# monatis/clip.cpp

Measured on AMD Instinct MI355X. Metric: image+text embeddings/sec, higher is better.
Workload: dtype f16

## Files before the change

### clip_cpp_amd/csrc/forward.cpp

```cpp
#include <cmath>
#include <cstdio>
#include <cstdlib>
#include <cstring>
#include <thread>
#include <utility>

#include "model.h"

namespace clipamd {

namespace {

constexpr size_t kGuardBytes = 4096;
constexpr int kGuardByte = 0xA5;
bool guard_mode() {
    static const bool on = [] { const char * e = getenv("CLIP_AMD_GUARD"); return e && e[0] == '1'; }();
    return on;
}

struct Carver {
    uint8_t * base;
    size_t off = 0;
    std::vector<size_t> * gaps = nullptr;
    explicit Carver(void * b, std::vector<size_t> * g = nullptr) : base((uint8_t *)b), gaps(g) { if (gaps) gaps->clear(); }
// ... 28 lines not shown
    std::vector<uint8_t> h(kGuardBytes);
    bool ok = true;
    for (size_t i = 0; i < ctx->guard_gaps.size(); i++) {
        if (hipMemcpy(h.data(), (uint8_t *)ctx->ws.base + ctx->guard_gaps[i], kGuardBytes, hipMemcpyDeviceToHost) != hipSuccess) return false;
        for (size_t k = 0; k < kGuardBytes; k++)
            if (h[k] != (uint8_t)kGuardByte) {
                fprintf(stderr, "%s: CLIP_AMD_GUARD: workspace buffer %zu was written %zu bytes past its end\n", who, i, k);
                ok = false;
                break;
            }
    }
    return ok;
}

struct ProfScope {
    clip_ctx * ctx;
    hipEvent_t a = nullptr, b = nullptr;
    bool on;
    std::string tag;
    double flops, bytes;
    ProfScope(clip_ctx * c, const char * family, long m, long n, long k, double fl, double by) : ctx(c), on(c->profiling), flops(fl), bytes(by) {
        if (!on) return;
        char buf[96];
        snprintf(buf, sizeof buf, "%s:%ldx%ldx%ld", family, m, n, k);
        tag = buf;
        (void)hipEventCreate(&a);
        (void)hipEventCreate(&b);
        (void)hipEventRecord(a, ctx->stream);
    }
    ~ProfScope() {
        if (!on) return;
        (void)hipEventRecord(b, ctx->stream);
        ctx->pending.push_back({a, b, tag, flops, bytes});
    }
};

double weight_bytes(const DevWeight & W) {
    const double nblk = (double)(W.K / 32) * W.N;
    switch (W.wtype) {
    case W_F16: return (double)W.N * W.K * 2;
    case W_Q4_0: return nblk * 18;
    case W_Q4_1: return nblk * 20;
    case W_Q5_0: return nblk * 22;
    case W_Q5_1: return nblk * 24;
    case W_Q8_0: return nblk * 34;
    case W_F32: return (double)W.N * W.K * 4;
    }
    return 0;
}

bool acts_f32(const clip_ctx * ctx, const DevTower & tw) {
    return ctx->f32_acts && !tw.layers.empty() && tw.layers[0].qkv.wtype == W_F32 && tw.layers[0].o.wtype == W_F32 && tw.layers[0].ff1.wtype == W_F32 && tw.layers[0].ff2.wtype == W_F32 &&
           tw.proj.wtype == W_F32;
}
void layernorm_act(bool f32, const float * x, int ldx, const int * in_rows, int in_row_mul, const float * w, const float * b, float eps, int rows, int h, half_t * dst,
                   hipStream_t s) {
    if (f32) launch_layernorm(x, ldx, in_rows, in_row_mul, w, b, eps, rows, h, nullptr, 0, (float *)dst, h, s);
    else launch_layernorm(x, ldx, in_rows, in_row_mul, w, b, eps, rows, h, dst, h, nullptr, 0, s);
}

bool device_shared(const clip_ctx * ctx) { return ctx->device_shared || ctx->sibling_busy || ctx->owner != nullptr; }

void gemm(clip_ctx * ctx, const char * what, const GemmParams & p0, int epi) {
    GemmParams p = p0;
    p.shared_device = device_shared(ctx);
    p.sk_ws = ctx->sk_ws; p.sk_ws_floats = ctx->sk_ws_floats; p.sk_cnt = ctx->sk_cnt; p.sk_cnt_n = ctx->sk_cnt_n;
    if (!ctx->profiling) {
        launch_gemm(p, epi, 0, ctx->stream);
        return;
    }
    const int wt = p.w16_pre ? (int)W_F16 : p.W.wtype;
    const int tile = gemm_tile_for(p.M, p.W.N, p.W.Kpad, wt != W_F16, p.shared_device);
    const bool panel = gemm_tile_uses_panel(tile) && wt == W_F16;
    const double fl = 2.0 * p.M * (double)p.W.N * p.W.K;
    const double wb = wt == W_F16 ? (double)p.W.N * p.W.K * 2 : weight_bytes(p.W);
    const double by = wb + (double)p.M * p.W.K * 2 + (double)p.M * p.W.N * (epi == EPI_F16 || epi == EPI_GELU_F16 || epi == EPI_QGELU_F16 ? 2 : epi == EPI_RESID_F32 ? 8 : 4)
                      + (p.xg_out ? (double)p.M * p.W.N * 2 : 0.0);
    char fam[96];
    if (wt == W_F32) snprintf(fam, sizeof fam, "gemm_f32_kernel<%d>/%s", epi, what);
    else if (panel && tile % 1000 == 261 && (epi == EPI_F16 || epi == EPI_GELU_F16 || epi == EPI_QGELU_F16)) snprintf(fam, sizeof fam, "gemm32_kernel<%d,4,%d>/%s", tile / 1000 == 320 ? 5 : 4, epi, what);
    else if (panel && tile % 1000 >= 259) snprintf(fam, sizeof fam, "gemm4_kernel<%d>/%s", epi, what);
    else if (panel) snprintf(fam, sizeof fam, "gemm8_kernel<%d,%d>/%s", tile / 32000, epi, what);
    else if (gemm_tile_is_ring(tile)) snprintf(fam, sizeof fam, "gemm_ring_kernel<%d,%d,4,%d,%d>/%s", wt, tile % 1000, tile % 1000 >= 128 ? 4 : 2, epi, what);
    else snprintf(fam, sizeof fam, "gemm_dma_kernel<%d,%d,%d,%d>/%s", wt, gemm_tile_uses_panel(tile) ? 160 : tile / 1000, gemm_tile_uses_panel(tile) ? 128 : tile % 1000, epi, what);
    ProfScope ps(ctx, fam, p.M, p.W.N, p.W.K, fl, by);
    launch_gemm(p, epi, 0, ctx->stream);
}

struct LayerPanels { const half_t * qkv = nullptr, * o = nullptr, * ff1 = nullptr, * ff2 = nullptr; };

bool ensure_panel(clip_ctx * ctx, size_t halfs) {
    if (ctx->w16_panel_halfs >= halfs) return true;
    (void)hipStreamSynchronize(ctx->stream);
    if (ctx->w16_panel) (void)hipFree(ctx->w16_panel);
    ctx->w16_panel = nullptr;
    ctx->w16_panel_halfs = 0;
    if (hipMalloc((void **)&ctx->w16_panel, halfs * sizeof(half_t)) != hipSuccess) { (void)hipGetLastError(); return false; }
    ctx->w16_panel_halfs = halfs;
    return true;
}

bool wants_resident_panel(const clip_ctx * ctx, const DevWeight & w, int i, int rows) {
    if (w.wtype == W_F16 || w.wtype == W_F32) return false;
    if (i == 3) return rows >= 4096 && gemm_tile_uses_panel(gemm_tile_for(rows, w.N, w.Kpad, false));
    if (i == 1) return rows >= 4096 && rows < 32768 && gemm_tile_uses_panel(gemm_tile_for(rows, w.N, w.Kpad, false));
    return rows >= 32768 && gemm_tile_for(rows, w.N, w.Kpad, false, device_shared(ctx)) % 1000 == 261;
}

LayerPanels dequant_layer(clip_ctx * ctx, const DevLayer & l, int rows, const half_t * const * res = nullptr) {
    LayerPanels lp;
    const DevWeight * ws[4] = {&l.qkv, &l.o, &l.ff1, &l.ff2};
    const half_t ** slot[4] = {&lp.qkv, &lp.o, &lp.ff1, &lp.ff2};
    const DevWeight * jw[4];
    half_t * jo[4];
    int nj = 0;
    size_t need = 0;
    bool todo[4];
    for (int i = 0; i < 4; i++) {
        if (res && res[i] && wants_resident_panel(ctx, *ws[i], i, rows)) { *slot[i] = res[i]; todo[i] = false; continue; }
        todo[i] = ws[i]->wtype != W_F16 && ws[i]->wtype != W_F32 && gemm_tile_uses_panel(gemm_tile_for(rows, ws[i]->N, ws[i]->Kpad, true));
        if (todo[i]) need += (size_t)ws[i]->Npad * ws[i]->Kpad;
    }
    if (!need || !ensure_panel(ctx, need)) return lp;
    size_t off = 0;
    for (int i = 0; i < 4; i++)
        if (todo[i]) {
            jw[nj] = ws[i];
            jo[nj] = ctx->w16_panel + off;
            *slot[i] = jo[nj];
            off += (size_t)ws[i]->Npad * ws[i]->Kpad;
            nj++;
        }
    ProfScope ps(ctx, "dequant_layer", rows, nj, 0, 0, (double)need * 2.5625);
    launch_dequant(jw, jo, nj, ctx->stream);
    return lp;
}

bool skinny_enabled() {
    static int on = -1;
    if (on < 0) { const char * e = getenv("CLIP_AMD_SKINNY"); on = !(e && e[0] == '0'); }
    return on != 0;
}

#ifdef CLIPAMD_SK_TIMING
unsigned long long * g_sk_stamps = nullptr;
int g_sk_stamp_launch = 0;
constexpr int SK_STAMP_LAUNCHES = 512;
#endif

void skinny(clip_ctx * ctx, const char * what, const SkinnyParams & p0, int epi) {
#ifdef CLIPAMD_SK_TIMING
    SkinnyParams p = p0;
    if (!g_sk_stamps && hipMalloc((void **)&g_sk_stamps, SK_STAMP_LAUNCHES * 16 * 8) == hipSuccess) (void)hipMemset(g_sk_stamps, 0, SK_STAMP_LAUNCHES * 16 * 8);
    if (g_sk_stamps) p.stamps = g_sk_stamps + (size_t)(g_sk_stamp_launch++ % SK_STAMP_LAUNCHES) * 16;
#else
    const SkinnyParams & p = p0;
#endif
    if (!ctx->profiling) { launch_skinny(p, epi, ctx->stream); return; }
    char fam[96];
    const int nw = (!p.x32 && p.W.Kpad >= 2048 && (epi == EPI_RESID_F32 || epi == EPI_PATCH_F32)) ? 8 : 4;
    snprintf(fam, sizeof fam, "skinny_kernel<%d,1,%d,%d,%s>/%s", p.W.wtype, nw, epi, p.x32 ? "true" : "false", what);
    const double fl = 2.0 * p.M * (double)p.W.N * p.W.K;
    const double by = weight_bytes(p.W) + (double)p.M * p.W.K * (p.x32 ? 4 : 2) + (double)p.M * p.W.N * (epi == EPI_RESID_F32 ? 8 : epi == EPI_F32 || epi == EPI_PATCH_F32 ? 4 : 2);
    ProfScope ps(ctx, fam, p.M, p.W.N, p.W.K, fl, by);
    launch_skinny(p, epi, ctx->stream);
}
// ... 767 lines not shown
```

### clip_cpp_amd/csrc/k_gemm.hip

```cpp

#include <vector>

#include "gemm_common.h"

namespace clipamd {

namespace {

constexpr int NTHREADS = 256;

constexpr bool gemm_tile_splits_k(int bm, int bn) { return bm == 64 && bn > 0; }

template <int WT, int BM, int BN, int EPI>
__global__ void __launch_bounds__(NTHREADS, ((BM + BN) * BK * 4 <= 80 * 1024 ? 2 : 1)) gemm_dma_kernel(const GemmParams p) {
    extern __shared__ __attribute__((aligned(16))) unsigned char smem_raw[];
    half_t * Xs = (half_t *)smem_raw;
    half_t * Ws = Xs + 2 * BM * BK;
    constexpr int TN = BN / 32, TM = BM / 32;
    constexpr int XPW = BM / 32;
    constexpr int WPW = BN / 32;

    const int tid = threadIdx.x;
    const int lane = tid & 63;
    const int wave = __builtin_amdgcn_readfirstlane(tid >> 6);
    const int wn = wave >> 1, wm = wave & 1;
    const int frow = lane & 15, fgrp = lane >> 4;

    const int tiles_m = (p.M + BM - 1) / BM;
    const int tiles_n = (p.W.N + BN - 1) / BN;
    constexpr bool SK = gemm_tile_splits_k(BM, BN);
    const int nwg = tiles_m * tiles_n * (SK ? p.ksplit : 1);
    int bid = blockIdx.x;
    {
        const int q = nwg >> 3, r = nwg & 7;
        const int xcd = bid & 7, idx = bid >> 3;
        bid = (xcd < r ? xcd * (q + 1) : r * (q + 1) + (xcd - r) * q) + idx;
    }
    const int ksplit = SK ? p.ksplit : 1;
    const int tile_id = SK ? bid / ksplit : bid;
    const int split = SK ? bid - tile_id * ksplit : 0;
    const int tile_n = tile_id % tiles_n, tile_m = tile_id / tiles_n;
    const int m0 = tile_m * BM, n0 = tile_n * BN;
    const int nk_all = p.W.Kpad / BK;
    const int kbeg = SK ? (split * nk_all) / ksplit : 0;
    const int nk = SK ? ((split + 1) * nk_all) / ksplit - kbeg : nk_all;
    const int last = nk - 1;

    const int prow = lane >> 3;
    const int pchunk = (lane & 7) ^ prow;
    const half_t * xsrc[XPW];
#pragma unroll
    for (int i = 0; i < XPW; i++) {
        int gm = m0 + (wave * XPW + i) * 8 + prow;
        gm = gm < p.M ? gm : p.M - 1;
        xsrc[i] = p.A + (size_t)gm * p.lda + pchunk * 8 + kbeg * BK;
    }
    const half_t * wsrc[WT == W_F16 ? WPW : 1];
    if constexpr (WT == W_F16) {
#pragma unroll
        for (int i = 0; i < WPW; i++)
            wsrc[i] = (const half_t *)p.W.w16 + (size_t)(n0 + (wave * WPW + i) * 8 + prow) * p.W.Kpad + pchunk * 8 + kbeg * BK;
    }
    constexpr int NB = (BN * 2 + NTHREADS - 1) / NTHREADS;
    RawBlock<WT> B0[NB], B1[NB];
    const int bnl = tid % BN, bkb = tid / BN;
    const bool bact = (BN * 2 >= NTHREADS) || tid < BN * 2;

#define DMA_TILE(buf_, kt_)                                                                    \
    {                                                                                          \
        _Pragma("unroll") for (int i = 0; i < XPW; i++)                                        \
            __builtin_amdgcn_global_load_lds((const __attribute__((address_space(1))) void *)(xsrc[i] + (kt_) * BK), \
                (__attribute__((address_space(3))) void *)(Xs + (buf_) * BM * BK + (wave * XPW + i) * 512), 16, 0, 0); \
        if constexpr (WT == W_F16) {                                                           \
            _Pragma("unroll") for (int i = 0; i < WPW; i++)                                    \
                __builtin_amdgcn_global_load_lds((const __attribute__((address_space(1))) void *)(wsrc[i] + (kt_) * BK), \
                    (__attribute__((address_space(3))) void *)(Ws + (buf_) * BN * BK + (wave * WPW + i) * 512), 16, 0, 0); \
        }                                                                                      \
    }
#define LOAD_B(B, kt_)                                                                         \
    if constexpr (WT != W_F16) {                                                               \
        if (bact) {                                                                            \
            _Pragma("unroll") for (int i_ = 0; i_ < NB; i_++)                                  \
                load_block<WT>(B[i_], p.W, (size_t)(((kt_) + kbeg) * 2 + bkb + i_ * (NTHREADS / BN)) * p.W.Npad + n0 + bnl); \
        }                                                                                      \
    }
#define STORE_B(B, buf_)                                                                       \
    if constexpr (WT != W_F16) {                                                               \
        if (bact) {                                                                            \
            half_t * wrow_ = Ws + (buf_) * BN * BK + bnl * BK;                                 \
            _Pragma("unroll") for (int i_ = 0; i_ < NB; i_++)                                  \
                _Pragma("unroll") for (int j = 0; j < 4; j++)                                  \
                    *(h8 *)(wrow_ + ((((bkb + i_ * (NTHREADS / BN)) * 4 + j) ^ (bnl & 7)) << 3)) = dequant_wfrag<WT>(block_word<WT>(B[i_], j), j); \
        }                                                                                      \
    }
    f4 acc[TN][TM];
#pragma unroll
    for (int a = 0; a < TN; a++)
#pragma unroll
// ... 127 lines not shown
    if (kt < nk) COMPUTE(0);
    }
#undef STEP_ILV
#undef FRAG
#undef DMA_TILE
#undef LOAD_B
#undef STORE_B
#undef COMPUTE
#undef COMPUTE_SCHED
    asm volatile("" ::: "memory");
#ifdef CLIPAMD_ABLATION
    if (p.debug & 8) {
        float keep = 0.f;
#pragma unroll
        for (int a = 0; a < TN; a++)
#pragma unroll
            for (int b = 0; b < TM; b++) keep += (acc[a][b][0] + acc[a][b][1]) + (acc[a][b][2] + acc[a][b][3]);
        if (keep == 1.2345e33f) ((float *)p.out)[tid] = keep;
        return;
    }
#endif
    if constexpr (SK) {
        if (ksplit > 1) {
            __shared__ int is_last;
            typedef unsigned long long u64;
            u64 * part = (u64 *)(p.sk_ws + ((size_t)tile_id * ksplit) * (BM * BN));
            constexpr int PER_SPLIT = BM * BN / 2;
#pragma unroll
            for (int a = 0; a < TN; a++)
#pragma unroll
                for (int b = 0; b < TM; b++) {
                    const float2 lo = make_float2(acc[a][b][0], acc[a][b][1]), hi = make_float2(acc[a][b][2], acc[a][b][3]);
                    u64 * dst = part + (size_t)split * PER_SPLIT + ((a * TM + b) * 2) * NTHREADS + tid;
                    __hip_atomic_store(dst, __builtin_bit_cast(u64, lo), __ATOMIC_RELAXED, __HIP_MEMORY_SCOPE_AGENT);
                    __hip_atomic_store(dst + NTHREADS, __builtin_bit_cast(u64, hi), __ATOMIC_RELAXED, __HIP_MEMORY_SCOPE_AGENT);
                }
            asm volatile("s_waitcnt vmcnt(0)" ::: "memory");
            __syncthreads();
            if (tid == 0) {
                const unsigned ticket = __hip_atomic_fetch_add(p.sk_cnt + tile_id, 1u, __ATOMIC_RELAXED, __HIP_MEMORY_SCOPE_AGENT);
                is_last = (ticket == (unsigned)ksplit - 1u);
                if (is_last) __hip_atomic_store(p.sk_cnt + tile_id, 0u, __ATOMIC_RELAXED, __HIP_MEMORY_SCOPE_AGENT);
            }
            __syncthreads();
            if (!is_last) return;
#pragma unroll
            for (int a = 0; a < TN; a++)
#pragma unroll
                for (int b = 0; b < TM; b++) acc[a][b] = (f4){0.f, 0.f, 0.f, 0.f};
            for (int sp = 0; sp < ksplit; sp++) {
#pragma unroll
                for (int a = 0; a < TN; a++)
#pragma unroll
                    for (int b = 0; b < TM; b++) {
                        const u64 * src = part + (size_t)sp * PER_SPLIT + ((a * TM + b) * 2) * NTHREADS + tid;
                        const float2 lo = __builtin_bit_cast(float2, __hip_atomic_load(src, __ATOMIC_RELAXED, __HIP_MEMORY_SCOPE_AGENT));
                        const float2 hi = __builtin_bit_cast(float2, __hip_atomic_load(src + NTHREADS, __ATOMIC_RELAXED, __HIP_MEMORY_SCOPE_AGENT));
                        acc[a][b] += (f4){lo.x, lo.y, hi.x, hi.y};
                    }
            }
        }
    }
    float2 * ln_rs = (float2 *)(smem_raw + ((BM * 272 + 15) & ~15));
    if constexpr (LNE) {
        if (ln) ln_rows_publish(ln_rs, ln_mine, tid, BM, [] { __syncthreads(); });
    }
    const float2 * rs_lane = ln_rs + wm * (BM / 2) + frow;
    if constexpr ((EPI == EPI_F16 || EPI == EPI_GELU_F16 || EPI == EPI_QGELU_F16) && BN == 128 && BM >= 128) {
        const int nb = n0 + wn * (BN / 2);
        if (nb + BN / 2 <= p.W.N && (p.ldc & 7) == 0) {
            if ((nk & 1) && !ln) __syncthreads();
            gemm_epilogue_f16_staged<EPI, TN, TM>(p, acc, nb, m0 + wm * (BM / 2), frow, fgrp, (half_t *)smem_raw + wave * (BM / 2) * 68, lane, ln, rs_lane);
            return;
        }
    }
    if constexpr (EPI == EPI_RESID_F32 && BN == 128 && BM >= 128) {
        if (p.xg_out) {
            if (nk & 1) __syncthreads();
            gemm_epilogue<EPI, TN, TM>(p, acc, n0 + wn * (BN / 2), m0 + wm * (BM / 2), frow, fgrp, false, rs_lane, (half_t *)smem_raw + wave * (BM / 2) * 68, lane);
            return;
        }
    }
    gemm_epilogue<EPI, TN, TM>(p, acc, n0 + wn * (BN / 2), m0 + wm * (BM / 2), frow, fgrp, ln, rs_lane);
}

template <int WT, int BM, int BN, int EPI>
void launch_dma(const GemmParams & p, hipStream_t stream) {
    const int tiles_m = (p.M + BM - 1) / BM, tiles_n = (p.W.N + BN - 1) / BN;
    constexpr size_t smem = (size_t)2 * (BM + BN) * BK * sizeof(half_t);
    static unsigned long long lds_ok = 0;
    if (smem > 64 * 1024) opt_in_dynamic_lds(gemm_dma_kernel<WT, BM, BN, EPI>, smem, lds_ok);
    int grid = tiles_m * tiles_n;
    if (gemm_tile_splits_k(BM, BN)) grid *= p.ksplit;
    hipLaunchKernelGGL((gemm_dma_kernel<WT, BM, BN, EPI>), dim3(grid), dim3(NTHREADS), smem, stream, p);
}

template <int WT, int EPI>
void launch_tile(const GemmParams & p, int tile, hipStream_t stream) {
    switch (tile % 1000000) {
    case 128128: launch_dma<WT, 128, 128, EPI>(p, stream); break;
    case 160128: launch_dma<WT, 160, 128, EPI>(p, stream); break;
    case 192128: launch_dma<WT, 192, 128, EPI>(p, stream); break;
#ifdef CLIPAMD_BIGTILES
    case 128256: launch_dma<WT, 128, 256, EPI>(p, stream); break;
    case 160256: launch_dma<WT, 160, 256, EPI>(p, stream); break;
    case 192256: launch_dma<WT, 192, 256, EPI>(p, stream); break;
    case 256256: launch_dma<WT, 256, 256, EPI>(p, stream); break;
#endif
    case 64128: launch_dma<WT, 64, 128, EPI>(p, stream); break;
    case 128064: launch_dma<WT, 128, 64, EPI>(p, stream); break;
    default: launch_dma<WT, 64, 64, EPI>(p, stream); break;
    }
}

template <int WT>
void launch_epi(const GemmParams & p, int epi, int tile, hipStream_t stream) {
    switch (epi) {
    case EPI_F32: launch_tile<WT, EPI_F32>(p, tile, stream); break;
    case EPI_F16: launch_tile<WT, EPI_F16>(p, tile, stream); break;
    case EPI_GELU_F16: launch_tile<WT, EPI_GELU_F16>(p, tile, stream); break;
    case EPI_QGELU_F16: launch_tile<WT, EPI_QGELU_F16>(p, tile, stream); break;
    case EPI_RESID_F32: launch_tile<WT, EPI_RESID_F32>(p, tile, stream); break;
    case EPI_PATCH_F32: launch_tile<WT, EPI_PATCH_F32>(p, tile, stream); break;
    }
}

int tile_override(int M, int N, int Kpad) {
#if !CLIPAMD_TEST_HOOKS
    (void)M; (void)N; (void)Kpad;
    return 0;
#else
    struct Ov { int M, N, K, tile; };
    static const std::vector<Ov> ovs = [] {
        std::vector<Ov> v;
        const char * e = getenv("CLIP_AMD_TILE_OVERRIDE");
        while (e && *e) {
            Ov o;
            int used = 0;
            if (sscanf(e, "%d,%d,%d,%d%n", &o.M, &o.N, &o.K, &o.tile, &used) == 4) v.push_back(o); else break;
            e += used;
            if (*e == ';') e++;
        }
        return v;
    }();
    for (const Ov & o : ovs) if (o.M == M && o.N == N && (o.K == 0 || o.K == Kpad)) return o.tile;
    return 0;
#endif
}

int pick_tile(int M, int N, int Kpad, bool quantised, bool shared = false) {
    auto wgs = [&](int bm, int bn) { return ((M + bm - 1) / bm) * ((N + bn - 1) / bn); };
    if (const int ov = tile_override(M, N, Kpad)) return ov;
    if (M <= 64) return 64064;
    if (M <= 4096) {
        const int tm = (M + 63) / 64, t64 = tm * ((N + 63) / 64), t128 = tm * ((N + 127) / 128), nk = Kpad / BK;
        if (nk < 32) {
            if (t64 <= 260) return 65064;
            if (t128 <= 500) return 65128;
        } else if (!quantised) {
            if (t64 <= 340) return 65064;
        } else if (M >= 1024 && t128 <= 340) {
            return 65128;
        }
    }
    if (wgs(128, 128) < 100) return wgs(64, 128) >= 256 ? 64128 : 64064;
    if (!shared && !quantised && M >= 32768 && N >= 3 * Kpad && (N & 63) == 0 && Kpad >= 128 && wgs(320, 256) >= 3 * 256) return 320261;
    if (M >= 32768 && wgs(256, 256) >= 2 * 256) return 256260;
    if (!shared && !quantised && M >= 8192 && N >= 2 * Kpad && (N & 63) == 0 && Kpad >= 128) {
        const int t4 = wgs(256, 256), t5 = wgs(320, 256);
        const int c4 = ((t4 + 255) / 256) * 256, c5 = ((t5 + 255) / 256) * 320;
        const bool five = c5 < c4;
        const int t = five ? t5 : t4;
        if ((float)t >= 0.8f * (float)(((t + 255) / 256) * 256)) return five ? 320261 : 256261;
    }
    if (!quantised && M >= 8192 && M < 32768 && N == Kpad && Kpad >= 512 && wgs(160, 256) >= 200 && wgs(160, 256) <= 256) return 160256;
    {
        const int t8 = wgs(160, 256);
        const float rounds = (float)t8 / 256.f;
        const float eff = rounds / ceilf(rounds);
        if (t8 >= 200 && eff >= 0.75f && (M >= 32768 || (Kpad >= 2048 && !quantised))) return 160256;
    }
    if (Kpad <= 512 && N <= 1536 && N >= 1024 && M >= 8192 && M <= 16384) return 192128;
    int best = 128128;
    float best_cost = 0.f;
    const int cand[4] = {128, 160, 192, 64};
    for (int bm : cand) {
        const float x = (float)wgs(bm, 128) / 512.f;
        const float g = x <= 0.5f ? 0.7f : x <= 1.f ? 1.f : 0.75f * x + 0.25f * ceilf(x);
        const float cost = g * (float)(bm + 32) * (bm == 64 ? 1.35f : 1.f);
        if (best_cost == 0.f || cost < best_cost) { best_cost = cost; best = bm * 1000 + 128; }
    }
    return best;
}

}

#ifdef CLIPAMD_GEMM_WT
#define CLIPAMD_CAT2(a, b) a##b
#define CLIPAMD_CAT(a, b) CLIPAMD_CAT2(a, b)
void CLIPAMD_CAT(launch_gemm_wt, CLIPAMD_GEMM_WT)(const GemmParams & p, int epilogue, int tile, hipStream_t stream) {
    launch_epi<CLIPAMD_GEMM_WT>(p, epilogue, tile, stream);
}
#else
void launch_gemm_wt0(const GemmParams &, int, int, hipStream_t);
void launch_gemm_wt1(const GemmParams &, int, int, hipStream_t);
void launch_gemm_wt2(const GemmParams &, int, int, hipStream_t);
void launch_gemm_wt3(const GemmParams &, int, int, hipStream_t);
void launch_gemm_wt4(const GemmParams &, int, int, hipStream_t);
void launch_gemm_wt5(const GemmParams &, int, int, hipStream_t);

int gemm_tile_for(int M, int N, int Kpad, bool quantised, bool shared_device) { return pick_tile(M, N, Kpad, quantised, shared_device); }

int gemm_fold_slotw(int tile) {
    tile %= 1000000;
    if (gemm_tile_is_ring(tile)) return 32;
    if (gemm_tile_uses_panel(tile)) return 64;
    return tile % 1000 == 64 ? 32 : 64;
}
static int fold_rest_tile(int M, int N, int Kpad, bool quantised) {
    const int t = pick_tile(M, N, Kpad, quantised);
    return gemm_fold_slotw(t) == 64 && t % 1000 != 258 && t % 1000 != 260 ? t : 64128;
}
int gemm_fold_slotw_for(int M, int N, int Kpad, bool quantised, bool shared_device) { return gemm_fold_slotw(pick_tile(M, N, Kpad, quantised, shared_device)); }

int pick_ksplit(int tiles, int nk) {
    if (nk < 8) return 1;
    int ks = (int)(sqrtf((float)nk / 1.5f) + 0.5f);
    if (tiles >= 256) ks = 1;
    if (tiles * ks > 1536) ks = 1536 / tiles;
    return ks < 1 ? 1 : ks > 16 ? 16 : ks;
}

int pick_ksplit_ring(int tiles, int nk, bool quantised) {
    if (nk < 32) return 1;
    if (quantised) return tiles <= 160 ? 3 : 1;
    return tiles <= 110 ? 2 : 1;
}

void launch_gemm(const GemmParams & p0, int epilogue, int tile, hipStream_t stream) {
    if (p0.M <= 0) return;
    if (p0.W.wtype == W_F32) {
        launch_gemm_f32(p0, epilogue, stream);
        return;
    }
    GemmParams p = p0;
    const bool heuristic = (tile == 0);
    int ksplit = tile / 1000000;
    tile %= 1000000;
    if (p.w16_pre && p.W.wtype != W_F16) {
        p.W.wtype = W_F16;
        p.W.w16 = p.w16_pre;
    }
    if (heuristic) {
        tile = pick_tile(p.M, p.W.N, p.W.Kpad, p.W.wtype != W_F16, p.shared_device);
        if (tile % 1000 == 261 && !gemm32_supported(p, epilogue)) tile = pick_tile(p.M, p.W.N, p.W.Kpad, p.W.wtype != W_F16, true);
    }
    if (tile % 1000 == 258 || tile % 1000 == 260) {
        const int tiles_n = (p.W.N + 255) / 256, tiles_m = (p.M + 255) / 256;
        const int mb = (int)(((long)tiles_m * tiles_n / 256) * 256 / tiles_n);
        tile = tile % 1000 == 258 ? 256256 : 256259;
        if (epilogue != EPI_PATCH_F32 && mb > 0 && mb < tiles_m) {
            const int m1 = mb * 256;
            const bool f16_out = epilogue == EPI_F16 || epilogue == EPI_GELU_F16 || epilogue == EPI_QGELU_F16;
            GemmParams head = p0, rest = p0;
            head.M = m1;
            rest.M = p.M - m1;
            rest.A = p.A + (size_t)m1 * p.lda;
            rest.out = (char *)p.out + (size_t)m1 * p.ldc * (f16_out ? sizeof(half_t) : sizeof(float));
            if (p.resid) rest.resid = p.resid + (size_t)m1 * p.ldc;
            if (p.ln_stats) rest.ln_stats = p.ln_stats + m1;
            if (p.ln_mu) rest.ln_mu = p.ln_mu + m1;
            if (p.mu_out) rest.mu_out = p.mu_out + m1;
            if (p.xg_mu) rest.xg_mu = p.xg_mu + m1;
            if (p.stats_out) rest.stats_out = p.stats_out + m1;
            if (p.xg_out) rest.xg_out = p.xg_out + (size_t)m1 * p.ldxg;
            launch_gemm(head, epilogue, tile, stream);
            launch_gemm(rest, epilogue, p.xg_out ? fold_rest_tile(rest.M, p.W.N, p.W.Kpad, p.W.wtype != W_F16) : 0, stream);
            return;
        }
    }
    if (gemm_tile_uses_panel(tile)) {
        const half_t * panel = p.W.wtype == W_F16 ? (const half_t *)p.W.w16 : p.w16_pre;
        if (!panel && p.w16_scratch && p.w16_scratch_halfs >= (size_t)p.W.Npad * p.W.Kpad) {
            const DevWeight * w = &p.W;
            half_t * o = p.w16_scratch;
            launch_dequant(&w, &o, 1, stream);
            panel = p.w16_scratch;
        }
        if (panel) {
            p.W.wtype = W_F16;
            p.W.w16 = panel;
            if (tile % 1000 == 261 ) {
                if (gemm32_supported(p, epilogue)) {
                    launch_gemm32(p, epilogue, tile / 1000 == 320 ? 5 : 4, stream);
                    return;
                }
                tile = 256259;
            }
            if (tile % 1000 == 259 && !p.xg_out) {
                launch_gemm4(p, epilogue, stream);
                return;
            }
            if (tile % 1000 == 259) tile = 256256;
            launch_gemm8(p, epilogue, tile / 32000, stream);
            return;
        }
        tile = 160128;
    }
    const bool ring = gemm_tile_is_ring(tile);
    const int bm = ring ? 64 : tile / 1000;
    int bn = tile % 1000;
    if (ring) bn = bn >= 128 ? 128 : 64;
    const int tiles = ((p.M + bm - 1) / bm) * ((p.W.N + bn - 1) / bn), nk = p.W.Kpad / BK;
    if (heuristic) ksplit = ring ? pick_ksplit_ring(tiles, nk, p.W.wtype != W_F16) : pick_ksplit(tiles, nk);
    if (ksplit < 1) ksplit = 1;
    if (!gemm_tile_splits_k(bm, bn) || !p.sk_ws || !p.sk_cnt || tiles > p.sk_cnt_n || p.no_splitk) ksplit = 1;
    if (ksplit > nk / 2) ksplit = nk / 2 > 0 ? nk / 2 : 1;
    while (ksplit > 1 && (size_t)tiles * ksplit * bm * bn > p.sk_ws_floats) ksplit--;
    p.ksplit = ksplit;
    if (ring) {
        launch_gemm_ring(p, epilogue, bn, stream);
        return;
    }
    switch (p.W.wtype) {
    case W_F16: launch_gemm_wt0(p, epilogue, tile, stream); break;
    case W_Q4_0: launch_gemm_wt1(p, epilogue, tile, stream); break;
    case W_Q4_1: launch_gemm_wt2(p, epilogue, tile, stream); break;
    case W_Q5_0: launch_gemm_wt3(p, epilogue, tile, stream); break;
    case W_Q5_1: launch_gemm_wt4(p, epilogue, tile, stream); break;
    case W_Q8_0: launch_gemm_wt5(p, epilogue, tile, stream); break;
    }
}
#endif

}
```

### clip_cpp_amd/csrc/kernels.h

```cpp
#pragma once

#include <hip/hip_runtime.h>
#include <cstdint>
#include <cstdio>

#include "jpeg_stages.h"

#ifndef CLIPAMD_TEST_HOOKS
#define CLIPAMD_TEST_HOOKS 1
#endif

namespace clipamd {

typedef _Float16 half_t;

template <typename K>
inline void opt_in_dynamic_lds(K kernel, size_t bytes, unsigned long long & done) {
    int dev = 0;
    (void)hipGetDevice(&dev);
    const unsigned long long bit = 1ull << (dev & 63);
    if (done & bit) return;
    const hipError_t e = hipFuncSetAttribute((const void *)kernel, hipFuncAttributeMaxDynamicSharedMemorySize, (int)bytes);
    if (e != hipSuccess) {
        fprintf(stderr, "clip (hip): hipFuncSetAttribute(MaxDynamicSharedMemorySize = %zu) failed: %s\n", bytes, hipGetErrorString(e));
        (void)hipGetLastError();
        return;
    }
    done |= bit;
}

enum WType : int { W_F16 = 0, W_Q4_0 = 1, W_Q4_1 = 2, W_Q5_0 = 3, W_Q5_1 = 4, W_Q8_0 = 5, W_F32 = 6 };

struct DevWeight {
    int wtype = W_F16;
    int N = 0, K = 0;
    int Npad = 0;
    int Kpad = 0;
    const void * qs = nullptr;
    const void * qh = nullptr;
    const void * dm = nullptr;
    const void * w16 = nullptr;
};

enum Epilogue : int {
    EPI_F32 = 0,
    EPI_F16 = 1,
    EPI_GELU_F16 = 2,
    EPI_QGELU_F16 = 3,
    EPI_RESID_F32 = 4,
    EPI_PATCH_F32 = 5,
    EPI_COUNT = 6
};

struct GemmParams {
    const half_t * A = nullptr;
    int lda = 0;
    int M = 0;
    DevWeight W;
    const float * bias = nullptr;
    void * out = nullptr;
    int ldc = 0;
    const float * resid = nullptr;
    float qscale = 1.0f;
    int qcols = 0;
    int Np = 0, T = 0;
    const float * pos = nullptr;
    float * sk_ws = nullptr;
    size_t sk_ws_floats = 0;
    unsigned * sk_cnt = nullptr;
    int sk_cnt_n = 0;
    int ksplit = 1;
    bool no_splitk = false;
    const half_t * w16_pre = nullptr;
    half_t * w16_scratch = nullptr;
    size_t w16_scratch_halfs = 0;
    int debug = 0;
    const float * ln_c = nullptr;
    const float2 * ln_stats = nullptr;
    int ln_slots = 0, ln_slotw = 0;
    int ln_stride = 0;
    float ln_eps = 0.f;
    half_t * xg_out = nullptr;
    int ldxg = 0;
    const float * xg_gamma = nullptr;
    float2 * stats_out = nullptr;
    int stats_stride = 0;
    const float * xg_mu = nullptr;
    const float * ln_mu = nullptr;
    float * mu_out = nullptr;
    bool shared_device = false;
    bool act_f32 = false;
};

void launch_gemm(const GemmParams & p, int epilogue, int tile, hipStream_t stream);
int gemm_tile_for(int M, int N, int Kpad, bool quantised, bool shared_device = false);
inline bool gemm_tile_is_ring(int tile) { return (tile % 1000000) / 1000 == 65; }
inline bool gemm_tile_uses_panel(int tile) { const int bn = tile % 1000; return !gemm_tile_is_ring(tile) && (bn == 256 || (bn >= 258 && bn <= 261)); }

void launch_gemm_ring(const GemmParams & p, int epilogue, int bn, hipStream_t stream);

void launch_gemm8(const GemmParams & p, int epilogue, int tm, hipStream_t stream);
void launch_gemm_f32(const GemmParams & p, int epilogue, hipStream_t stream);
void launch_gemm4(const GemmParams & p, int epilogue, hipStream_t stream);
bool gemm32_supported(const GemmParams & p, int epilogue);
void launch_gemm32(const GemmParams & p, int epilogue, int form, hipStream_t stream);
struct DequantJobs { DevWeight W[4]; half_t * out[4]; int blk_end[4]; int n = 0; };
void launch_dequant(const DevWeight * const * ws, half_t * const * outs, int n, hipStream_t stream);

int gemm_fold_slotw(int tile);
int gemm_fold_slotw_for(int M, int N, int Kpad, bool quantised, bool shared_device = false);
void launch_fold_vectors(const DevWeight & W, const float * gamma, const float * beta, const float * bias, float * c_out, float * b_out,
                         hipStream_t stream);

struct SkinnyParams {
    const half_t * A16 = nullptr;
    int lda = 0;
    const float * x32 = nullptr;
    int ldx = 0;
    const float * ln_w = nullptr, * ln_b = nullptr;
    float eps = 0.f;
    const float2 * stats_in = nullptr;
    int stats_slots = 0;
    int M = 0;
    DevWeight W;
    const float * bias = nullptr;
    void * out = nullptr;
    int ldc = 0;
    const float * resid = nullptr;
    float qscale = 1.0f;
    int qcols = 0;
    int Np = 0, T = 0;
    const float * pos = nullptr;
    float2 * stats_out = nullptr;
    int stats_cap = 128;
    const float * ln_c = nullptr;
    const float2 * fstats = nullptr;
    int fslots = 0, fslotw = 0, fstride = 0;
    half_t * xg_out = nullptr;
    int ldxg = 0;
    const float * xg_gamma = nullptr;
    float2 * fstats_out = nullptr;
    int fstride_out = 0;
    const float * xg_mu = nullptr, * ln_mu = nullptr;
    float * mu_out = nullptr;
    unsigned long long * stamps = nullptr;
};
constexpr int SKINNY_MAX_ROWS = 512;
bool skinny_supported(const SkinnyParams & p, int epilogue);
void launch_skinny(const SkinnyParams & p, int epilogue, hipStream_t stream);
void launch_row_stats(const float * x, int ldx, int rows, int h, float2 * stats, hipStream_t stream);

void launch_layernorm(const float * x, int ldx, const int * in_rows, int in_row_mul, const float * w, const float * b, float eps,
                      int rows, int h, half_t * out16, int ld16, float * out32, int ld32, hipStream_t stream);
void launch_layernorm_prep(const float * x, int ldx, const float * w, const float * b, float eps, int rows, int h, float * out32, int ld32,
                           const float * gamma_next, half_t * xg, int ldxg, float2 * stats, hipStream_t stream, float * mu_out = nullptr,
                           const float * class_embd = nullptr, const float * pos0 = nullptr, int T = 0);

bool launch_attention(const half_t * qkv, half_t * out, int nseq, int T_uniform, const int * seq_start, int max_len,
                      int h, int n_head, bool causal, hipStream_t stream);
int attention_whole_row_max_len(int d_head);
bool launch_attention_whole_row(const half_t * qkv, half_t * out, int nseq, int T_uniform, const int * seq_start, int max_len,
                                int h, int n_head, bool causal, hipStream_t stream);
bool launch_attention_long(const half_t * qkv, half_t * out, int nseq, int T_uniform, const int * seq_start, int max_len,
                           int h, int n_head, bool causal, hipStream_t stream);

bool launch_attention_f32(const float * qkv, float * out, int nseq, int T_uniform, const int * seq_start, int max_len,
                          int h, int n_head, bool causal, hipStream_t stream);

void launch_im2col(const void * imgs, bool imgs_f16, half_t * col, int B, int S, int P, int Kpad, hipStream_t stream);

void launch_gather_rows(const float * x, const half_t * a, const int * in_rows, int in_row_mul, int rows, int h, float * xp, half_t * ap, hipStream_t stream);

void launch_cls_rows(float * x, const float * class_embd, const float * pos, int B, int T, int h, hipStream_t stream);

void launch_meta_upload(const int * src_mapped, int * seq, int * last, int n_texts, unsigned * done_mapped, unsigned stamp, hipStream_t stream);
void launch_text_embed(const int32_t * ids, const int * seq_start, int nseq, int rows, const void * tok_raw,
                       int tok_type, const float * pos, int h, float * x, hipStream_t stream,
                       const float * gamma_next = nullptr, half_t * xg = nullptr, int ldxg = 0, float2 * stats = nullptr, float * mu_out = nullptr);

void launch_l2norm(const float * v, float * out, int rows, int n, bool normalize, hipStream_t stream);
// ... 148 lines not shown
```

Before: 125,300.

## Add wide 256-column GEMM tile for block-quantised weights with fp16 epilogues

Adds a specialised GEMM body with 128/160x256 tiles for quantised weights. It keeps the dequantised weight fragment single-buffered in LDS, double-buffers activations through direct global-to-LDS loads, and splits accumulators between AGPRs and VGPRs. The tile picker selects it for large-M, wide-N quantised GEMMs on shared devices, to raise weight and activation reuse per workgroup. Unsupported cases fall back to the narrow tiles. The trade-off is higher register and LDS pressure and extra code complexity.

```diff
diff --git a/clip_cpp_amd/csrc/forward.cpp b/clip_cpp_amd/csrc/forward.cpp
--- a/clip_cpp_amd/csrc/forward.cpp
+++ b/clip_cpp_amd/csrc/forward.cpp
@@ -134,6 +134,11 @@
     else if (panel && tile % 1000 >= 259) snprintf(fam, sizeof fam, "gemm4_kernel<%d>/%s", epi, what);
     else if (panel) snprintf(fam, sizeof fam, "gemm8_kernel<%d,%d>/%s", tile / 32000, epi, what);
     else if (gemm_tile_is_ring(tile)) snprintf(fam, sizeof fam, "gemm_ring_kernel<%d,%d,4,%d,%d>/%s", wt, tile % 1000, tile % 1000 >= 128 ? 4 : 2, epi, what);
+    else if (gemm_tile_is_wide(tile)) {
+        const bool wide = wt != W_F16 && (epi == EPI_F16 || epi == EPI_GELU_F16 || epi == EPI_QGELU_F16) && !p.xg_out;
+        const int t = wide ? tile : gemm_tile_for_narrow(p.M, p.W.N, p.W.Kpad, wt != W_F16, p.shared_device);
+        snprintf(fam, sizeof fam, "gemm_dma_kernel<%d,%d,%d,%d>/%s", wt, wide ? ((wt == W_Q5_0 || wt == W_Q8_0) ? 128 : tile / 1000) : gemm_tile_uses_panel(t) ? 160 : t / 1000, wide ? 256 : gemm_tile_uses_panel(t) ? 128 : t % 1000, epi, what);
+    }
     else snprintf(fam, sizeof fam, "gemm_dma_kernel<%d,%d,%d,%d>/%s", wt, gemm_tile_uses_panel(tile) ? 160 : tile / 1000, gemm_tile_uses_panel(tile) ? 128 : tile % 1000, epi, what);
     ProfScope ps(ctx, fam, p.M, p.W.N, p.W.K, fl, by);
     launch_gemm(p, epi, 0, ctx->stream);
diff --git a/clip_cpp_amd/csrc/gemm_wide.h b/clip_cpp_amd/csrc/gemm_wide.h
--- /dev/null
+++ b/clip_cpp_amd/csrc/gemm_wide.h
@@ -0,0 +1,155 @@
+#pragma once
+
+#include "gemm_common.h"
+
+namespace clipamd {
+
+namespace {
+
+constexpr int WIDE_BN = 256;
+constexpr size_t gemm_wide_lds_bytes(int bm) { return (size_t)2 * bm * BK * 2 + (size_t)WIDE_BN * BK * 2 + (size_t)bm * 8; }
+constexpr bool gemm_wide_epilogue(int epi) { return epi == EPI_F16 || epi == EPI_GELU_F16 || epi == EPI_QGELU_F16; }
+constexpr bool gemm_wide_bm_fits(int wt, int bm) { return bm == 128 || (bm == 160 && (wt == W_Q4_0 || wt == W_Q4_1 || wt == W_Q5_1)); }
+
+template <int WT, int BM, int EPI>
+__device__ __forceinline__ void gemm_wide_body(const GemmParams & p, unsigned char * smem_raw) {
+    static_assert(WT != W_F16 && gemm_wide_bm_fits(WT, BM) && gemm_wide_epilogue(EPI), "wide tile: block-quantised weights, fp16 outputs");
+    constexpr int BN = WIDE_BN, TN = 8, TM = BM / 32, XPW = BM / 32, HM = BM / 2;
+    half_t * Xs = (half_t *)smem_raw;
+    half_t * Ws = Xs + 2 * BM * BK;
+    float2 * ln_rs = (float2 *)(Ws + BN * BK);
+
+    const int tid = threadIdx.x;
+    const int lane = tid & 63;
+    const int wave = __builtin_amdgcn_readfirstlane(tid >> 6);
+    const int wn = wave >> 1, wm = wave & 1;
+    const int frow = lane & 15, fgrp = lane >> 4;
+
+    const int tiles_m = (p.M + BM - 1) / BM;
+    const int tiles_n = (p.W.N + BN - 1) / BN;
+    const int nwg = tiles_m * tiles_n;
+    int bid = blockIdx.x;
+    {
+        const int q = nwg >> 3, r = nwg & 7;
+        const int xcd = bid & 7, idx = bid >> 3;
+        bid = (xcd < r ? xcd * (q + 1) : r * (q + 1) + (xcd - r) * q) + idx;
+    }
+    const int tile_n = bid % tiles_n, tile_m = bid / tiles_n;
+    const int m0 = tile_m * BM, n0 = tile_n * BN;
+    const int nk = p.W.Kpad / BK;
+    const int last = nk - 1;
+
+    const int prow = lane >> 3;
+    const int xrow0 = m0 + wave * XPW * 8 + prow;
+    const unsigned xcol = (unsigned)(((lane & 7) ^ prow) * 8);
+    const int mlast = p.M - 1;
+    RawBlock<WT> R0, R1;
+    const int wrow_g = n0 + tid < p.W.Npad ? n0 + tid : p.W.Npad - 1;
+    constexpr int WOFF = 2 * BM * BK * 2;
+    const int wst = WOFF + tid * 128 + ((tid & 7) << 4);
+    const int fsw = (fgrp ^ (frow & 7)) << 4;
+    const int lw = WOFF + (wn * 128 + frow) * 128 + fsw;
+    const int lx = (wm * HM + frow) * 128 + fsw;
+#define WIDE_LOAD(R_, kt_, s_) load_block<WT>(R_, p.W, (size_t)((kt_) * 2 + (s_)) * p.W.Npad + wrow_g)
+#define WIDE_STORE_WORD(R_, s_, j_) *(h8 *)(smem_raw + (wst ^ (((s_) * 4 + (j_)) << 4))) = dequant_wfrag<WT>(block_word<WT>(R_, (j_)), (j_))
+#define WIDE_DMA(buf_, kt_, i_)                                                                                   \
+    {                                                                                                             \
+        const int gm_ = xrow0 + (i_) * 8 < mlast ? xrow0 + (i_) * 8 : mlast;                                      \
+        const unsigned xo_ = (unsigned)gm_ * (unsigned)p.lda + xcol + (unsigned)((kt_) * BK);                     \
+        __builtin_amdgcn_global_load_lds((const __attribute__((address_space(1))) void *)(p.A + xo_),             \
+            (__attribute__((address_space(3))) void *)(Xs + (buf_) * BM * BK + (wave * XPW + (i_)) * 512), 16, 0, 0); \
+    }
+#define WIDE_WFRAG(S_, a_) (*(const h8 *)(smem_raw + ((S_) ? (lw ^ 64) : lw) + (a_) * 2048))
+#define WIDE_XFRAG(xb_, S_, b_) (*(const h8 *)(smem_raw + (xb_) * BM * BK * 2 + ((S_) ? (lx ^ 64) : lx) + (b_) * 2048))
+
+    constexpr int NACC_A = 32;
+#define WIDE_PIN_ACC()                                                                                            \
+    _Pragma("unroll") for (int a = 0; a < TN; a++)                                                                \
+        _Pragma("unroll") for (int b = 0; b < TM; b++) {                                                          \
+            if (a * TM + b < NACC_A) asm volatile("" : "+a"(acc[a][b])); else asm volatile("" : "+v"(acc[a][b])); \
+        }
+    f4 acc[TN][TM];
+#pragma unroll
+    for (int a = 0; a < TN; a++)
+#pragma unroll
+        for (int b = 0; b < TM; b++) acc[a][b] = (f4){0.f, 0.f, 0.f, 0.f};
+
+    constexpr int NM = TN * TM, GS = 2, NG = NM / GS;
+    static_assert(NM % GS == 0 && NG >= 8, "groups");
+#define WIDE_PHASE(S_, xb_, DMA_, dkt_, RL_, lkt_, RS_)                                                           \
+    {                                                                                                             \
+        h8 wf[TN], xf[TM];                                                                                        \
+        wf[0] = WIDE_WFRAG(S_, 0);                                                                                \
+        _Pragma("unroll") for (int b = 0; b < TM; b++) xf[b] = WIDE_XFRAG(xb_, S_, b);                            \
+        _Pragma("unroll") for (int a = 1; a < TN / 2; a++) wf[a] = WIDE_WFRAG(S_, a);                             \
+        WIDE_LOAD(RL_, lkt_, S_);                                                                                 \
+        __builtin_amdgcn_sched_barrier(0);                                                                        \
+        _Pragma("unroll") for (int g = 0; g < NG; g++) {                                                          \
+            _Pragma("unroll") for (int i = 0; i < GS; i++) {                                                      \
+                const int idx = g * GS + i;                                                                       \
+                if (idx < NACC_A) asm volatile("v_mfma_f32_16x16x32_f16 %0, %1, %2, %0" : "+a"(acc[idx / TM][idx % TM]) : "v"(wf[idx / TM]), "v"(xf[idx % TM])); \
+                else asm volatile("v_mfma_f32_16x16x32_f16 %0, %1, %2, %0" : "+v"(acc[idx / TM][idx % TM]) : "v"(wf[idx / TM]), "v"(xf[idx % TM])); \
+            }                                                                                                     \
+            _Pragma("unroll") for (int a = TN / 2; a < TN; a++)      \
+                if (g == (TM * (a - TN / 2) + TM - 1) / GS) wf[a] = WIDE_WFRAG(S_, a);                            \
+            if (DMA_) {                                                                                           \
+                _Pragma("unroll") for (int pc = 0; pc < XPW; pc++)                                                \
+                    if (g == (pc * NG) / XPW) WIDE_DMA((xb_) ^ 1, dkt_, pc)                                      \
+            }                                                                                                     \
+            _Pragma("unroll") for (int wd = 0; wd < 4; wd++)                                                      \
+                if (g == (wd * NG) / 4 + 1) WIDE_STORE_WORD(RS_, (S_) ^ 1, wd);                                   \
+            __builtin_amdgcn_sched_barrier(0);                                                                    \
+        }                                                                                                         \
+    }
+#define WIDE_STEP(xb_, kt_)                                                                                       \
+    {                                                                                                             \
+        const int kn_ = (kt_) + 1 < last ? (kt_) + 1 : last;                                                      \
+        WIDE_PHASE(0, xb_, true, kn_, R0, kn_, R1);                                                               \
+        __syncthreads();                                                                                          \
+        WIDE_PHASE(1, xb_, false, 0, R1, kn_, R0);                                                                \
+        __syncthreads();                                                                                          \
+    }
+
+#pragma unroll
+    for (int i = 0; i < XPW; i++) WIDE_DMA(0, 0, i)
+    WIDE_LOAD(R0, 0, 0);
+    WIDE_LOAD(R1, 0, 1);
+    const bool ln = p.ln_c != nullptr;
+    if (ln && tid < BM) ln_rs[tid] = ln_row_centred(p, m0 + tid < p.M ? m0 + tid : p.M - 1, tile_n == 0);
+    WIDE_PIN_ACC();
+    asm volatile("s_nop 7\n\ts_nop 7" ::: "memory");
+#pragma unroll
+    for (int j = 0; j < 4; j++) WIDE_STORE_WORD(R0, 0, j);
+    __syncthreads();
+    int kt = 0;
+    for (; kt + 1 < nk; kt += 2) {
+        WIDE_STEP(0, kt);
+        WIDE_STEP(1, kt + 1);
+    }
+    if (kt < nk) WIDE_STEP(0, kt);
+#undef WIDE_STEP
+#undef WIDE_PHASE
+#undef WIDE_WFRAG
+#undef WIDE_XFRAG
+#undef WIDE_DMA
+#undef WIDE_STORE_WORD
+#undef WIDE_LOAD
+    asm volatile("s_nop 15\n\ts_nop 15" ::: "memory");
+    WIDE_PIN_ACC();
+#undef WIDE_PIN_ACC
+
+    const int nb = n0 + wn * 128, mb = m0 + wm * HM;
+    const float2 * rs_lane = ln_rs + wm * HM + frow;
+    half_t * stage = (half_t *)smem_raw + wave * HM * 68;
+    typedef f4 half_acc_t[4][TM];
+#pragma unroll
+    for (int hf = 0; hf < 2; hf++) {
+        half_acc_t & hacc = *(half_acc_t *)&acc[4 * hf];
+        if (nb + 64 * hf + 64 <= p.W.N && (p.ldc & 7) == 0) gemm_epilogue_f16_staged<EPI, 4, TM>(p, hacc, nb + 64 * hf, mb, frow, fgrp, stage, lane, ln, rs_lane);
+        else gemm_epilogue<EPI, 4, TM>(p, hacc, nb + 64 * hf, mb, frow, fgrp, ln, rs_lane);
+    }
+}
+
+}
+
+}
diff --git a/clip_cpp_amd/csrc/k_gemm.hip b/clip_cpp_amd/csrc/k_gemm.hip
--- a/clip_cpp_amd/csrc/k_gemm.hip
+++ b/clip_cpp_amd/csrc/k_gemm.hip
@@ -2,6 +2,7 @@
 #include <vector>
 
 #include "gemm_common.h"
+#include "gemm_wide.h"
 
 namespace clipamd {
 
@@ -10,10 +11,18 @@
 constexpr int NTHREADS = 256;
 
 constexpr bool gemm_tile_splits_k(int bm, int bn) { return bm == 64 && bn > 0; }
+constexpr bool gemm_tile_is_wide_inst(int wt, int bm, int bn, int epi) { return bn == WIDE_BN && wt != W_F16 && gemm_wide_bm_fits(wt, bm) && gemm_wide_epilogue(epi); }
+constexpr size_t gemm_dma_lds_bytes(int wt, int bm, int bn, int epi) {
+    return gemm_tile_is_wide_inst(wt, bm, bn, epi) ? gemm_wide_lds_bytes(bm) : (size_t)2 * (bm + bn) * BK * sizeof(half_t);
+}
 
 template <int WT, int BM, int BN, int EPI>
-__global__ void __launch_bounds__(NTHREADS, ((BM + BN) * BK * 4 <= 80 * 1024 ? 2 : 1)) gemm_dma_kernel(const GemmParams p) {
+__global__ void __launch_bounds__(NTHREADS, (gemm_dma_lds_bytes(WT, BM, BN, EPI) <= 80 * 1024 ? 2 : 1)) gemm_dma_kernel(const GemmParams p) {
     extern __shared__ __attribute__((aligned(16))) unsigned char smem_raw[];
+    if constexpr (gemm_tile_is_wide_inst(WT, BM, BN, EPI)) {
+        gemm_wide_body<WT, BM, EPI>(p, smem_raw);
+        return;
+    } else {
     half_t * Xs = (half_t *)smem_raw;
     half_t * Ws = Xs + 2 * BM * BK;
     constexpr int TN = BN / 32, TM = BM / 32;
@@ -307,12 +316,13 @@
         }
     }
     gemm_epilogue<EPI, TN, TM>(p, acc, n0 + wn * (BN / 2), m0 + wm * (BM / 2), frow, fgrp, ln, rs_lane);
+    }
 }
 
 template <int WT, int BM, int BN, int EPI>
 void launch_dma(const GemmParams & p, hipStream_t stream) {
     const int tiles_m = (p.M + BM - 1) / BM, tiles_n = (p.W.N + BN - 1) / BN;
-    constexpr size_t smem = (size_t)2 * (BM + BN) * BK * sizeof(half_t);
+    constexpr size_t smem = gemm_dma_lds_bytes(WT, BM, BN, EPI);
     static unsigned long long lds_ok = 0;
     if (smem > 64 * 1024) opt_in_dynamic_lds(gemm_dma_kernel<WT, BM, BN, EPI>, smem, lds_ok);
     int grid = tiles_m * tiles_n;
@@ -326,6 +336,12 @@
     case 128128: launch_dma<WT, 128, 128, EPI>(p, stream); break;
     case 160128: launch_dma<WT, 160, 128, EPI>(p, stream); break;
     case 192128: launch_dma<WT, 192, 128, EPI>(p, stream); break;
+    case 128257: if constexpr (gemm_tile_is_wide_inst(WT, 128, 256, EPI)) launch_dma<WT, 128, 256, EPI>(p, stream); else launch_dma<WT, 160, 128, EPI>(p, stream); break;
+    case 160257:
+        if constexpr (gemm_tile_is_wide_inst(WT, 160, 256, EPI)) launch_dma<WT, 160, 256, EPI>(p, stream);
+        else if constexpr (gemm_tile_is_wide_inst(WT, 128, 256, EPI)) launch_dma<WT, 128, 256, EPI>(p, stream);
+        else launch_dma<WT, 160, 128, EPI>(p, stream);
+        break;
 #ifdef CLIPAMD_BIGTILES
     case 128256: launch_dma<WT, 128, 256, EPI>(p, stream); break;
     case 160256: launch_dma<WT, 160, 256, EPI>(p, stream); break;
@@ -373,9 +389,9 @@
 #endif
 }
 
-int pick_tile(int M, int N, int Kpad, bool quantised, bool shared = false) {
+int pick_tile(int M, int N, int Kpad, bool quantised, bool shared = false, bool wide_ok = true) {
     auto wgs = [&](int bm, int bn) { return ((M + bm - 1) / bm) * ((N + bn - 1) / bn); };
-    if (const int ov = tile_override(M, N, Kpad)) return ov;
+    if (const int ov = tile_override(M, N, Kpad); ov && (wide_ok || !gemm_tile_is_wide(ov))) return ov;
     if (M <= 64) return 64064;
     if (M <= 4096) {
         const int tm = (M + 63) / 64, t64 = tm * ((N + 63) / 64), t128 = tm * ((N + 127) / 128), nk = Kpad / BK;
@@ -405,6 +421,10 @@
         const float eff = rounds / ceilf(rounds);
         if (t8 >= 200 && eff >= 0.75f && (M >= 32768 || (Kpad >= 2048 && !quantised))) return 160256;
     }
+    if (wide_ok && quantised && shared && M >= 8192 && M < 32768 && N >= 4 * Kpad && (N & 255) == 0) {
+        const int t = wgs(160, 256), rounds = (t + 511) / 512;
+        if (10 * t >= 9 * 512 * rounds) return 160257;
+    }
     if (Kpad <= 512 && N <= 1536 && N >= 1024 && M >= 8192 && M <= 16384) return 192128;
     int best = 128128;
     float best_cost = 0.f;
@@ -435,6 +455,7 @@
 void launch_gemm_wt5(const GemmParams &, int, int, hipStream_t);
 
 int gemm_tile_for(int M, int N, int Kpad, bool quantised, bool shared_device) { return pick_tile(M, N, Kpad, quantised, shared_device); }
+int gemm_tile_for_narrow(int M, int N, int Kpad, bool quantised, bool shared_device) { return pick_tile(M, N, Kpad, quantised, shared_device, false); }
 
 int gemm_fold_slotw(int tile) {
     tile %= 1000000;
@@ -460,6 +481,10 @@
     if (nk < 32) return 1;
     if (quantised) return tiles <= 160 ? 3 : 1;
     return tiles <= 110 ? 2 : 1;
+}
+
+static bool gemm_wide_supported(const GemmParams & p, int epilogue) {
+    return p.W.wtype != W_F16 && p.W.wtype != W_F32 && gemm_wide_epilogue(epilogue) && !p.xg_out && (size_t)p.M * (size_t)p.lda < ((size_t)1 << 31);
 }
 
 void launch_gemm(const GemmParams & p0, int epilogue, int tile, hipStream_t stream) {
@@ -479,7 +504,9 @@
     if (heuristic) {
         tile = pick_tile(p.M, p.W.N, p.W.Kpad, p.W.wtype != W_F16, p.shared_device);
         if (tile % 1000 == 261 && !gemm32_supported(p, epilogue)) tile = pick_tile(p.M, p.W.N, p.W.Kpad, p.W.wtype != W_F16, true);
-    }
+        if (gemm_tile_is_wide(tile) && !gemm_wide_supported(p, epilogue)) tile = pick_tile(p.M, p.W.N, p.W.Kpad, p.W.wtype != W_F16, p.shared_device, false);
+    }
+    if (gemm_tile_is_wide(tile) && !gemm_wide_supported(p, epilogue)) tile = 160128;
     if (tile % 1000 == 258 || tile % 1000 == 260) {
         const int tiles_n = (p.W.N + 255) / 256, tiles_m = (p.M + 255) / 256;
         const int mb = (int)(((long)tiles_m * tiles_n / 256) * 256 / tiles_n);
@@ -536,6 +563,7 @@
     const int bm = ring ? 64 : tile / 1000;
     int bn = tile % 1000;
     if (ring) bn = bn >= 128 ? 128 : 64;
+    if (gemm_tile_is_wide(tile)) bn = WIDE_BN;
     const int tiles = ((p.M + bm - 1) / bm) * ((p.W.N + bn - 1) / bn), nk = p.W.Kpad / BK;
     if (heuristic) ksplit = ring ? pick_ksplit_ring(tiles, nk, p.W.wtype != W_F16) : pick_ksplit(tiles, nk);
     if (ksplit < 1) ksplit = 1;
diff --git a/clip_cpp_amd/csrc/kernels.h b/clip_cpp_amd/csrc/kernels.h
--- a/clip_cpp_amd/csrc/kernels.h
+++ b/clip_cpp_amd/csrc/kernels.h
@@ -96,6 +96,8 @@
 int gemm_tile_for(int M, int N, int Kpad, bool quantised, bool shared_device = false);
 inline bool gemm_tile_is_ring(int tile) { return (tile % 1000000) / 1000 == 65; }
 inline bool gemm_tile_uses_panel(int tile) { const int bn = tile % 1000; return !gemm_tile_is_ring(tile) && (bn == 256 || (bn >= 258 && bn <= 261)); }
+inline bool gemm_tile_is_wide(int tile) { return !gemm_tile_is_ring(tile) && tile % 1000 == 257; }
+int gemm_tile_for_narrow(int M, int N, int Kpad, bool quantised, bool shared_device);
 
 void launch_gemm_ring(const GemmParams & p, int epilogue, int bn, hipStream_t stream);
 
```

New measurement: 127,100 (median of 6 runs). 1.4% higher.
